# CCIG-Champalimaud/adell-mri

Hardware: AMD Instinct MI355X
Metric: volumes/sec 3D U-Net 128^3 2-ch seg (train step: fwd+loss+bwd+SGD) (higher is better)
Workload: dtype f32 (f16x3 split MFMA, fp32 accumulate); 1 GPU; BASELINE configs[1]: u-net-3d-resnet.yaml UNetPL, 2x128^3, batch 2/GPU, dice+focal, SGD-Nesterov; per_gpu_batch=2, parallelism=dp1, yaml=configs/u-net-3d-resnet.yaml, built_by=parse_config_unet -> get_segmentation_network('unet'), gradient_exchange=none (1 rank)

## Files before the change

adell_mri_amd/_lib.py:

```python
import ctypes
import os

_HERE = os.path.dirname(os.path.abspath(__file__))
LIB_PATH = os.environ.get("ADELL_HIP_LIBRARY") or os.path.join(_HERE, "libadellhip.so")

_lib = None

OK = 0
E_BADARG, E_UNSUPPORTED, E_HIP, E_NOMEM = -1, -2, -3, -4

ACT_IDS = {
    "identity": 0, "swish": 1, "silu": 1, "relu": 2, "leaky_relu": 3, "prelu": 4,
    "gelu": 5, "sigmoid": 6, "tanh": 7, "elu": 8,
}


class AdellHipError(RuntimeError):
    pass


class ConvDesc(ctypes.Structure):
    _fields_ = [(n, ctypes.c_int32) for n in (
        "N", "D", "H", "W", "C0", "C1", "Cout", "KD", "KH", "KW", "SD", "SH", "SW",
        "PD", "PH", "PW", "Do", "Ho", "Wo")]
# ... 65 lines not shown
    "adell_bn_running_update": (_i, [_vp] * 5 + [_i, _l, _f, _f, _vp]),
    "adell_bn_stats_sums": (_i, [_vp, _i, _i, _i, _l, _vp, _vp, ctypes.c_size_t, _vp]),
    "adell_bn_stats_from_sums": (_i, [_vp, _i, _f, _vp, _vp, _vp, _vp, _vp, _f, _vp]),
    "adell_channel_partials_ntiles": (_i, [_l]),
    "adell_channel_partials": (_i, [_vp, _i, _l, _i, _vp, _vp]),
    "adell_norm_act_fwd": (_i, [ctypes.POINTER(NormActDesc), _vp, _vp, _vp, _vp, _vp, _vp, _vp, _vp]),
    "adell_norm_act_mask_bytes": (_l, [ctypes.POINTER(NormActDesc)]),
    "adell_norm_act_fwd_split": (_i, [ctypes.POINTER(NormActDesc)] + [_vp] * 7 + [_i, _vp, _vp]),
    "adell_split_rows_from_f32": (_i, [_vp, _i, _l, _i, _vp, _vp, _vp]),
    "adell_split_rows_to_f32": (_i, [_vp, _i, _l, _i, _vp, _vp, _vp]),
    "adell_conv3d_f16x3_rows_ok": (_i, [ctypes.POINTER(ConvDesc)]),
    "adell_conv3d_bwd_weight_f16x3_rows_ok": (_i, [ctypes.POINTER(ConvDesc)]),
    "adell_conv3d_bwd_weight_f16x3_plan": (_i, [ctypes.POINTER(ConvDesc), _vp]),
    "adell_conv3d_bwd_weight_f16x3_rows": (_i, [ctypes.POINTER(ConvDesc)] + [_vp] * 10
                                           + [ctypes.c_size_t, _vp]),
    "adell_conv3d_fwd_f16x3_rows": (_i, [ctypes.POINTER(ConvDesc)] + [_vp] * 10 + [_i, _vp, _vp]),
    "adell_norm_act_fwd_mask": (_i, [ctypes.POINTER(NormActDesc)] + [_vp] * 9),
    "adell_norm_act_bwd_from_dt": (_i, [ctypes.POINTER(NormActDesc)] + [_vp] * 5 + [_i, _i, _i, _vp, _vp,
                                                                              ctypes.c_size_t, _vp]),
    "adell_conv3d_bwd_data_f16x3_adn_ntiles": (_i, [ctypes.POINTER(ConvDesc)]),
    "adell_conv3d_bwd_data_f16x3_adn": (_i, [ctypes.POINTER(ConvDesc)] + [_vp] * 7
                                        + [ctypes.POINTER(AdnSite), ctypes.POINTER(AdnSite), _vp, _i, _vp]),
    "adell_norm_act_bwd_workspace": (_l, [ctypes.POINTER(NormActDesc)]),
    "adell_norm_act_bwd": (_i, [ctypes.POINTER(NormActDesc)] + [_vp] * 11 + [ctypes.c_size_t, _vp]),
    "adell_norm_act_plan": (_i, [ctypes.POINTER(NormActDesc)] + [_i] * 6 + [_vp]),
    "adell_norm_act_stats_plan": (_i, [_i, _i, _i, _vp]),
    "adell_norm_act_bwd_sums": (_i, [ctypes.POINTER(NormActDesc)] + [_vp] * 11 + [ctypes.c_size_t, _vp]),
    "adell_norm_act_bwd_apply_sums": (_i, [ctypes.POINTER(NormActDesc)] + [_vp] * 10
                                      + [ctypes.c_size_t, _vp]),
    "adell_norm_act_bwd_lowrank": (_i, [ctypes.POINTER(NormActDesc), _vp, _vp, _vp, _i, _vp, _vp, _vp,
# ... 185 lines not shown
    "adell_lesion_candidates_capacity": (_l, [_i] * 6),
    "adell_lesion_candidates": (_i, [_vp, _l, _i, _i, _i, _i, _f, _f] + [_i] * 5 + [_vp] * 6
                                + [_l, ctypes.POINTER(ctypes.c_int), _vp, _l, _vp]),
    "adell_item_stats_workspace": (_l, [_i, _l]),
    "adell_item_stats": (_i, [_vp, _i, _l, _vp, _vp, ctypes.c_size_t, _vp]),
    "adell_aug_intensity": (_i, [_vp, _vp, _i, _l, _vp, ctypes.c_uint64, ctypes.c_uint32, _vp]),
    "adell_affine_sample": (_i, [_vp, _vp, _i, _i, _i, _i, _i, _vp, _i, _i, _vp]),
    "adell_axis_filter": (_i, [_vp, _vp, _i, _i, _i, _i, _i, _i, _vp, _i, _vp]),
    "adell_bias_field": (_i, [_vp, _vp, _i, _i, _i, _i, _i, _vp, _vp]),
    "adell_axis_lut_sample": (_i, [_vp, _vp, _i, _i, _i, _i, _i, _vp, _i, _vp]),
    "adell_dw_mfma_ok": (_i, [_i] * 8 + [_vp, _vp]),
    "adell_dw_dense_ok": (_i, [_i] * 8 + [_vp, _vp]),
    "adell_dw_wgrad_mfma_ok": (_i, [_i] * 8 + [_vp, _vp]),
    "adell_dwconv3d_plan": (_i, [_i] * 11 + [_vp]),
    "adell_wgrad_zring_plan": (_i, [_i] * 16 + [_vp]),
    "adell_rowscale_fwd": (_i, [_vp] * 5 + [_i, _i, _vp]),
    "adell_rowscale_bwd": (_i, [_vp] * 8 + [_i, _i, _vp]),
    "adell_window_ndhwc": (_i, [_vp, _vp] + [_i] * 11 + [_vp]),
    "adell_gibbs_workspace": (_l, [_i, _i, _i, _i, _i]),
    "adell_gibbs_lowpass": (_i, [_vp, _vp, _i, _i, _i, _i, _i, _vp, _vp, ctypes.c_size_t, _vp]),
    "adell_gather_nd": (_i, [_vp, _vp, _i, _vp, _vp, _vp, _i, _vp, _vp, _vp, _vp]),
    "adell_layernorm_rows_fwd": (_i, [_vp, _l, _i, _i, _l, _l, _vp, _vp, _f, _vp, _vp, _vp, _vp]),
    "adell_layernorm_rows_bwd_workspace": (_l, [_l, _i]),
    "adell_layernorm_rows_bwd": (_i, [_vp, _vp, _vp, _vp, _vp, _l, _i, _i, _l, _l, _vp, _l, _l,
                                      _vp, _vp, _vp, ctypes.c_size_t, _vp]),
    "adell_winattn_fwd": (_i, [_vp, _vp, _vp, _l, _l, _vp, _vp, _i, _l, _i, _i, _i, _i, _f, _f,
                               ctypes.c_ulong, ctypes.c_uint, _vp, _vp, _vp]),
    "adell_winattn_bwd": (_i, [_vp, _vp, _vp, _l, _l, _vp, _vp, _i, _vp, _vp, _vp, _l, _i, _i, _i,
                               _i, _f, _f, ctypes.c_ulong, ctypes.c_uint, _vp, _vp, _vp, _vp, _vp]),
    "adell_gemm_f32_workspace_floats": (_l, [_i, _i, _i]),
# ... 73 lines not shown
```

adell_mri_amd/csrc/common.h:

```cpp
#pragma once
#include <hip/hip_runtime.h>
#include <stdint.h>
#include <stdio.h>
#include "../../include/adell_hip.h"

typedef float f32x16 __attribute__((ext_vector_type(16)));
typedef float f32x4 __attribute__((ext_vector_type(4)));

#define ADELL_WAVE 64
#define ADELL_GLOBAL __attribute__((address_space(1)))

void adell_set_error(const char* fmt, ...);

struct AdellTuning {
  int igemm_nospec;
  int igemm_no8;
  int no_splitk;
  int wgrad_nozring;
  int attn_nomfma;
  int dw_nomfma;
  int dw_wgrad_nomfma;
  int wgrad_no16;
  int igemm_no16;
  int gemm_norows;
// ... 19 lines not shown
      adell_set_error("%s:%d: %s -> %s", __FILE__, __LINE__, #expr,            \
                      hipGetErrorString(_e));                                  \
      return ADELL_E_HIP;                                                      \
    }                                                                          \
  } while (0)

#define ADELL_REQUIRE(cond, ...)                                               \
  do {                                                                         \
    if (!(cond)) {                                                             \
      adell_set_error(__VA_ARGS__);                                            \
      return ADELL_E_BADARG;                                                   \
    }                                                                          \
  } while (0)

constexpr int kAdellLdsPerCu = 160 * 1024;

template <auto Kern, typename... Args>
static int adell_launch(dim3 grid, dim3 block, size_t lds, hipStream_t st, const Args&... args) {
  static const hipError_t attr = [] {
    hipFuncAttributes fa;
    const hipError_t e = hipFuncGetAttributes(&fa, reinterpret_cast<const void*>(Kern));
    if (e != hipSuccess) return e;
    return hipFuncSetAttribute(reinterpret_cast<const void*>(Kern),
                               hipFuncAttributeMaxDynamicSharedMemorySize,
                               kAdellLdsPerCu - (int)fa.sharedSizeBytes);
  }();
  if (attr != hipSuccess) {
    adell_set_error("%s: raising the dynamic LDS limit -> %s", __PRETTY_FUNCTION__,
                    hipGetErrorString(attr));
    return ADELL_E_HIP;
  }
  hipLaunchKernelGGL(Kern, grid, block, lds, st, args...);
  const hipError_t e = hipGetLastError();
  if (e != hipSuccess) {
    adell_set_error("%s: launch -> %s", __PRETTY_FUNCTION__, hipGetErrorString(e));
    return ADELL_E_HIP;
  }
  return ADELL_OK;
}

int adell_cu_count();
// ... 125 lines not shown
```

adell_mri_amd/csrc/conv3d.hip:

```cpp
#include "conv_igemm.h"
#include "conv_igemm_f16.h"

#ifdef ADELL_DEBUG
__device__ unsigned long long* adell_g_stamps = nullptr;
extern "C" int adell_debug_set_stamps(void* device_buffer) {
  ADELL_CHECK_HIP(hipMemcpyToSymbol(HIP_SYMBOL(adell_g_stamps), &device_buffer, sizeof(void*)));
  return ADELL_OK;
}
#endif

struct ConvTile {
  int cfg;
  int BM, BN;
  int lTX, lTY, lTZ;
};

static void adell_shape_brick(int BM, int Wo, int Ho, int Do, int* lx, int* ly,
                              int* lz) {
  int bits = adell_ilog2(BM);
  int cap[3] = {adell_ilog2(Wo), adell_ilog2(Ho), adell_ilog2(Do)};
  int l[3] = {0, 0, 0};
  int pref[3] = {3, 3, 2};
  for (int pass = 0; pass < 2 && bits > 0; ++pass) {
    bool progress = true;
// ... 352 lines not shown
  int rows_ok;
  int adn_rows;
  int stat_rows;
  dim3 grid;
};

static bool adell_is_3s1(const ConvArgs& a) {
  return a.KD == 3 && a.KH == 3 && a.KW == 3 && a.SD == 1 && a.SH == 1 && a.SW == 1 && a.UPS == 1 &&
         a.UPSY == 1 && a.UPSZ == 1 && a.shuffle == 0;
}

static bool adell_item_below_4g(const ConvArgs& a) {
  return (size_t)a.D * a.H * a.W * (a.C0 > a.C1 ? a.C0 : a.C1) < ((size_t)1 << 30);
}

static int adell_plan_tile_f16(const ConvArgs& a, int N, ConvPlanF16* p) {
  ConvTile t = adell_pick_tile(N, a.Do, a.Ho, a.Wo, a.Cout, g_conv_force_cfg);
  const bool is3s1 = adell_is_3s1(a);
  if (g_conv_force_cfg < 0 && adell_conv_zring16_ok(&a)) {
    int seglen = 0, nseg = 0;
    adell_conv_zring16_segments(N, a.Do, a.Ho, a.Wo, &seglen, &nseg);
    t.cfg = 8;
    t.BM = 64;
    t.BN = 16;
    t.lTX = 3; t.lTY = 3; t.lTZ = 0;
    p->tile = t;
    p->brick = {adell_cdiv(a.Wo, 8), adell_cdiv(a.Ho, 8), nseg, 10, 10, seglen, 100};
    p->GKH = 3;
    p->lds = 0;
    return ADELL_OK;
// ... 37 lines not shown
    const int next = t.cfg == 0 ? 2 : t.cfg == 1 ? 3 : 6;
    if (t.cfg == next || g_conv_force_cfg >= 0) break;
    t = adell_pick_tile(N, a.Do, a.Ho, a.Wo, a.Cout, next);
  }
  if (lds > 160 * 1024) {
    adell_set_error("conv f16x3: LDS need %zu B exceeds 160 KiB (k=%d stride=%d)", lds, a.KW, a.SW);
    return ADELL_E_UNSUPPORTED;
  }
  if (t.cfg == 1 && !retiled && is3s1 && t.lTX == 3 && t.lTY == 3 && t.lTZ == 2 && a.Do >= 8 &&
      a.C0 % 16 == 0 && a.C1 % 16 == 0 && adell_item_below_4g(a) && g_conv_force_cfg < 0 &&
      !g_adell_tune.igemm_nospec && !g_adell_tune.igemm_no8) {
    t.cfg = 4;
    t.BM = 512;
    t.lTZ = 3;
    p->brick = adell_brick(a, t);
    lds = (size_t)1000 * 64 + (size_t)7 * 32 * 64 + 64;
  }
  if (a.shuffle != 0 && a.KD == 1 && a.KH == 1 && a.KW == 1 && a.Cout >= 128 &&
      g_conv_force_cfg < 0 && !g_adell_tune.igemm_nospec) {
    t.cfg = 5;
    t.BM = 64;
    t.BN = 256;
    adell_shape_brick(64, a.Wo, a.Ho, a.Do, &t.lTX, &t.lTY, &t.lTZ);
    p->brick = adell_brick(a, t);
    p->GKH = 1;
    lds = (size_t)p->brick.VP * 64 + (size_t)256 * 64 + 64;
    if (lds < (size_t)1 * 256 * 2 * sizeof(float)) lds = (size_t)256 * 2 * sizeof(float);
  }
  p->tile = t;
  p->lds = lds;
  return ADELL_OK;
// ... 504 lines not shown
```

adell_mri_amd/csrc/conv_wgrad_f16.hip:

```cpp
#include "conv_wgrad_host.h"

typedef _Float16 half8 __attribute__((ext_vector_type(8)));
typedef _Float16 half4 __attribute__((ext_vector_type(4)));
typedef __fp16 fp16x4 __attribute__((__vector_size__(4 * sizeof(__fp16))));

__device__ __forceinline__ half8 adell_tr_frag(const char* base, int off, int step) {
  typedef __attribute__((address_space(3))) fp16x4* lds_p;
  const fp16x4 lo4 = __builtin_amdgcn_ds_read_tr16_b64_v4f16((lds_p)(base + off));
  const fp16x4 hi4 = __builtin_amdgcn_ds_read_tr16_b64_v4f16((lds_p)(base + off + step));
  half8 r;
  r[0] = (_Float16)lo4[0]; r[1] = (_Float16)lo4[1]; r[2] = (_Float16)lo4[2]; r[3] = (_Float16)lo4[3];
  r[4] = (_Float16)hi4[0]; r[5] = (_Float16)hi4[1]; r[6] = (_Float16)hi4[2]; r[7] = (_Float16)hi4[3];
  return r;
}

struct WgradF16Args {
  const float* x0;
  const float* x1;
  const float* dy;
  float* ws;
  float* wsdb;
  const unsigned* xmax;
  const unsigned* ymax;
  int N, D, H, W;
// ... 498 lines not shown
  a.PD = d.PD; a.PH = d.PH; a.PW = d.PW;
  a.Do = d.Do; a.Ho = d.Ho; a.Wo = d.Wo;
  a.lTY = p.lTY; a.ntx = p.ntx; a.nty = p.nty; a.HX = p.HX; a.HY = p.HY;
  a.GKH = p.GKH; a.NGY = p.NGY;
  a.TCI = p.TCI; a.TCO = p.TCO; a.nci = p.nci; a.nco = p.nco; a.R = p.R;
  a.ksplit = p.ksplit;
  a.vecx = (d.C0 % 4 == 0) && (d.C1 % 4 == 0) && (((uintptr_t)x0 & 15) == 0) &&
           (((uintptr_t)x1 & 15) == 0);
  a.vecy = (d.Cout % 4 == 0) && (((uintptr_t)dy & 15) == 0);
  return r.inst->launch(a, r.grid, p.lds, st);
}

static int adell_wgrad_f16_run(const adell_conv3d_desc& d, const float* x0, const float* x1,
                               const float* dy, float* out, float* db, const uint32_t* xmax_in,
                               const uint32_t* ymax_in, void* ws, size_t ws_bytes, hipStream_t st,
                               const int* xk0 = nullptr, const int* xk1 = nullptr) {
  WgradRoute r;
  const int prc = adell_wgrad_route(d, &r);
  ADELL_REQUIRE((!xk0 && !xk1) || r.rows_ok,
                "wgrad f16x3: this problem does not take split-row sources "
                "(adell_conv3d_bwd_weight_f16x3_rows_ok)");
  if (prc != ADELL_OK) return prc;
  if (r.route == ADELL_WGRAD_SMALL)
    return adell_wgrad_small(&d, x0, x1, dy, out, db, ws, ws_bytes, st);
  const int Cin = d.C0 + d.C1, Cout = d.Cout, ntap = d.KD * d.KH * d.KW;
  const size_t need = adell_wgrad_f16_ws(r.R, d);
  ADELL_REQUIRE(ws != nullptr && ws_bytes >= need, "wgrad f16x3: workspace too small (%zu < %zu)",
                ws_bytes, need);
  float* slabs = (float*)ws;
  float* wsdb = slabs + (size_t)r.R * ntap * Cin * Cout;
  unsigned* amax = reinterpret_cast<unsigned*>(wsdb + (size_t)r.R * Cout);
// ... 2 lines not shown
  auto blocks_for = [](long n) { long b = (n / 4 + 255) / 256; return (int)(b > 2048 ? 2048 : (b < 1 ? 1 : b)); };
  if (!xmax_in || !ymax_in) ADELL_CHECK_HIP(hipMemsetAsync(amax, 0, 4 * sizeof(unsigned), st));
  if (!xmax_in) {
    if (!xk0)
      hipLaunchKernelGGL(adell_absmax2_kernel, dim3(blocks_for(nx0)), dim3(256), 0, st, x0, nx0, amax);
    if (d.C1 > 0 && !xk1)
      hipLaunchKernelGGL(adell_absmax2_kernel, dim3(blocks_for(nx1)), dim3(256), 0, st, x1, nx1, amax);
  }
  if (!ymax_in)
    hipLaunchKernelGGL(adell_absmax2_kernel, dim3(blocks_for(ny)), dim3(256), 0, st, dy, ny, amax + 1);
  const unsigned* xmax = xmax_in ? xmax_in : amax;
  const unsigned* ymax = ymax_in ? ymax_in : amax + 1;
  float* dbs = db ? wsdb : nullptr;
  int rc;
  if (r.route == ADELL_WGRAD_ZRING32 || r.route == ADELL_WGRAD_ZRING16)
    rc = adell_wgrad_zring_launch(d, r.zr, x0, x1, dy, slabs, dbs, xmax, ymax, st, xk0, xk1);
  else if (r.route == ADELL_WGRAD_S2)
    rc = adell_wgrad_s2_launch(d, r.s2, x0, dy, slabs, dbs, xmax, ymax, st);
  else
    rc = adell_wgrad_plane_launch(d, r, x0, x1, dy, slabs, dbs, xmax, ymax, st);
  if (rc != ADELL_OK) return rc;
  return adell_wgrad_reduce_launch(slabs, out, r.R, ntap, Cin, Cout, dbs, db, st);
}

extern "C" long adell_conv3d_bwd_weight_f16x3_workspace(const adell_conv3d_desc* d) {
  if (!d) return ADELL_E_BADARG;
  WgradRoute r;
  if (adell_wgrad_route(*d, &r) != ADELL_OK) return ADELL_E_UNSUPPORTED;
  return adell_wgrad_f16_workspace(*d, r);
}

// ... 18 lines not shown
    for (int i = 0; i < 8; ++i) out[16 + i] = v[i];
  }
  WgradPlan p32;
  if (r.route != ADELL_WGRAD_SMALL && adell_wgrad_plan(*d, &p32) == ADELL_OK) out[24] = p32.maxj_inst;
  return ADELL_OK;
}

extern "C" int adell_conv3d_bwd_weight_f16x3(const adell_conv3d_desc* d, const float* x0,
                                             const float* x1, const float* dy, float* dw,
                                             float* db, const uint32_t* x_absmax,
                                             const uint32_t* dy_absmax, void* workspace,
                                             size_t workspace_bytes, void* stream) {
  ADELL_REQUIRE(d && x0 && dy && dw, "conv_bwd_weight_f16x3: null pointer");
  ADELL_REQUIRE(d->C1 == 0 || x1, "conv_bwd_weight_f16x3: C1 > 0 needs x1");
  return adell_wgrad_f16_run(*d, x0, x1, dy, dw, db, x_absmax, dy_absmax, workspace,
                             workspace_bytes, (hipStream_t)stream);
}

extern "C" int adell_conv3d_bwd_weight_f16x3_rows_ok(const adell_conv3d_desc* d) {
  WgradRoute r;
  return d && adell_wgrad_route(*d, &r) == ADELL_OK && r.rows_ok ? 1 : 0;
}

extern "C" int adell_conv3d_bwd_weight_f16x3_rows(const adell_conv3d_desc* d, const void* x0,
                                                  const int* xk0, const void* x1, const int* xk1,
                                                  const float* dy, float* dw, float* db,
                                                  const uint32_t* x_absmax,
                                                  const uint32_t* dy_absmax, void* workspace,
                                                  size_t workspace_bytes, void* stream) {
  ADELL_REQUIRE(d && x0 && dy && dw, "conv_bwd_weight_f16x3_rows: null pointer");
  ADELL_REQUIRE(d->C1 == 0 || x1, "conv_bwd_weight_f16x3_rows: C1 > 0 needs x1");
  ADELL_REQUIRE(xk0 || xk1, "conv_bwd_weight_f16x3_rows: no split-row source");
  return adell_wgrad_f16_run(*d, (const float*)x0, (const float*)x1, dy, dw, db, x_absmax,
                             dy_absmax, workspace, workspace_bytes, (hipStream_t)stream, xk0, xk1);
}
```

adell_mri_amd/csrc/conv_wgrad_host.h:

```cpp
#pragma once
#include "common.h"

struct WgradZrPlan {
  int ntx, nty, nseg, seglen, nci, nco, R, t16;
};
bool adell_wgrad_zring_plan_desc(const adell_conv3d_desc& d, WgradZrPlan& p);
int adell_wgrad_zring_launch(const adell_conv3d_desc& d, const WgradZrPlan& p, const float* x0,
                             const float* x1, const float* dy, float* slabs, float* wsdb,
                             const unsigned* xmax, const unsigned* ymax, hipStream_t st,
                             const int* xk0, const int* xk1);

struct WgradS2Plan {
  int ntx, nty, ntz, nbricks, blocks, R;
};
bool adell_wgrad_s2_plan(const adell_conv3d_desc& d, WgradS2Plan& p);
int adell_wgrad_s2_launch(const adell_conv3d_desc& d, const WgradS2Plan& p, const float* x,
                          const float* dy, float* slabs, float* wsdb, const unsigned* xmax,
                          const unsigned* ymax, hipStream_t st);

struct WgradF16Plan {
  int lTY, HX, HY, TCI, TCO, nci, nco, maxj, R, ntx, nty, GKH, NGY, ksplit;
  size_t lds;
};

struct WgradPlan {
// ... 14 lines not shown
```

adell_mri_amd/csrc/conv_wgrad_zring.hip:

```cpp
#include "conv_wgrad_host.h"

typedef _Float16 zr_half8 __attribute__((ext_vector_type(8)));
typedef _Float16 zr_half4 __attribute__((ext_vector_type(4)));
typedef __fp16 zr_fp16x4 __attribute__((__vector_size__(4 * sizeof(__fp16))));

__device__ __forceinline__ zr_half8 adell_zr_frag(const char* p) {
  typedef __attribute__((address_space(3))) zr_fp16x4* lds_p;
  const zr_fp16x4 lo4 = __builtin_amdgcn_ds_read_tr16_b64_v4f16((lds_p)(p));
  const zr_fp16x4 hi4 = __builtin_amdgcn_ds_read_tr16_b64_v4f16((lds_p)(p + 4 * 32));
  zr_half8 r;
  r[0] = (_Float16)lo4[0]; r[1] = (_Float16)lo4[1]; r[2] = (_Float16)lo4[2]; r[3] = (_Float16)lo4[3];
  r[4] = (_Float16)hi4[0]; r[5] = (_Float16)hi4[1]; r[6] = (_Float16)hi4[2]; r[7] = (_Float16)hi4[3];
  return r;
}

struct WgradZrArgs {
  const float* x0;
  const float* x1;
  const float* dy;
  float* ws;
  float* wsdb;
  const unsigned* xmax;
  const unsigned* ymax;
  const int* xk0;
// ... 557 lines not shown
  p.R = (int)(nunits < target ? nunits : target);
  return true;
}

extern "C" int adell_wgrad_zring_plan(int N, int D, int H, int W, int C0, int C1, int Cout, int KD,
                                      int KH, int KW, int SD, int SH, int SW, int Do, int Ho, int Wo,
                                      int* plan) {
  const adell_conv3d_desc d = {N, D, H, W, C0, C1, Cout, KD, KH, KW, SD, SH, SW, 0, 0, 0, Do, Ho, Wo};
  WgradZrPlan p;
  if (!adell_wgrad_zring_plan_desc(d, p)) return 0;
  const int v[8] = {p.ntx, p.nty, p.nseg, p.seglen, p.nci, p.nco, p.R, p.t16};
  for (int i = 0; i < 8; ++i) plan[i] = v[i];
  return 1;
}

int adell_wgrad_zring_launch(const adell_conv3d_desc& d, const WgradZrPlan& p, const float* x0,
                             const float* x1, const float* dy, float* slabs, float* wsdb,
                             const unsigned* xmax, const unsigned* ymax, hipStream_t st,
                             const int* xk0, const int* xk1) {
  WgradZrArgs a = {};
  a.x0 = x0; a.x1 = x1; a.dy = dy; a.ws = slabs; a.wsdb = wsdb; a.xmax = xmax; a.ymax = ymax;
  a.xk0 = xk0; a.xk1 = xk1;
  a.N = d.N; a.D = d.D; a.H = d.H; a.W = d.W; a.C0 = d.C0; a.C1 = d.C1; a.Cin = d.C0 + d.C1;
  a.Cout = d.Cout;
  a.PD = d.PD; a.PH = d.PH; a.PW = d.PW; a.Do = d.Do; a.Ho = d.Ho; a.Wo = d.Wo;
  a.ntx = p.ntx; a.nty = p.nty; a.nseg = p.nseg; a.seglen = p.seglen;
  a.nci = p.nci; a.nco = p.nco; a.R = p.R;
  a.dbg = g_adell_tune.zr_dbg;
  const dim3 grid((unsigned)p.R, (unsigned)(p.nci * p.nco));
  if (p.t16) {
    const size_t lds16 = 2 * (ZR_SLOTS * (size_t)Z16_XPLANE + 2 * (size_t)Z16_YPLANE);
    hipLaunchKernelGGL(adell_conv_wgrad_zring16_kernel, grid, dim3(256), lds16, st, a);
    ADELL_CHECK_HIP(hipGetLastError());
    return ADELL_OK;
  }
  const size_t lds = ZR_SLOTS * (size_t)ZR_PLANE + 2 * (size_t)ZR_YBUF;
  return adell_launch<adell_conv_wgrad_zring_kernel>(grid, dim3(256), lds, st, a);
}
```

adell_mri_amd/functional.py:

```python
import collections
import ctypes
import itertools
import os
import weakref

import numpy as np
import torch
import torch.distributed as dist

from . import _lib, ops

_dropout_counter = itertools.count(1)

CONV_PRECISION = os.environ.get("ADELL_CONV_PRECISION", "f16x3")
FLAGS = {"s2class_always": bool(os.environ.get("ADELL_S2CLASS_ALWAYS")),
         "no_s2class": bool(os.environ.get("ADELL_NO_S2CLASS")),
         "no_fold": bool(os.environ.get("ADELL_NO_FOLD")),
         "no_adn_fuse": bool(os.environ.get("ADELL_NO_ADN_FUSE")),
         "no_lowrank": bool(os.environ.get("ADELL_NO_LOWRANK")),
         "wgrad_stream": os.environ.get("ADELL_WGRAD_STREAM", "1") != "0",
         "no_rows": bool(os.environ.get("ADELL_NO_ROWS")),
         "no_pointwise_gemm": bool(os.environ.get("ADELL_NO_POINTWISE_GEMM")),
         "no_seq_attention": bool(os.environ.get("ADELL_NO_SEQ_ATTENTION")),
         "no_mlp_fuse": not bool(os.environ.get("ADELL_MLP_FUSE")),
         "mlp_min_elems": int(os.environ.get("ADELL_MLP_MIN_ELEMS", str(1 << 20))),
         "no_cinfold_wgrad_f16": bool(os.environ.get("ADELL_NO_CINFOLD_WGRAD_F16"))}


def set_conv_precision(mode):
    global CONV_PRECISION
    if mode not in ("f16x3", "fp32"):
        raise ValueError("conv precision must be 'f16x3' or 'fp32'")
    CONV_PRECISION = mode
    _sync_dw_precision()

# ... 533 lines not shown
                    if site is not None:
                        site.fused, site.part, site.poff = True, part, poff
            else:
                fused = add0 is not None and C1 == 0 and f16x3
                dx0, dx1 = ops.conv3d_bwd_data(dy, wpb, in_size, C0, C1, k, stride, padding,
                                               amax=dy_amax, add0=add0 if fused else None)
                if fused:
                    add0 = None
        elif route is not None:
            raise ValueError(f"conv3d: unknown backward-data route {route!r}")
        dx0 = dx0 if need[0] else None
        dx1 = dx1 if x1 is not None and need[1] else None
        want_db = has_bias and need[3]
        wroute = conv3d_wgrad_route(call.route, need[2], want_db)

        def weight_grads():
            db = None
            if wroute == "conv1_small":
                dw, db = ops.conv1_small_bwd_weight(x0, x1, dy, want_db)
            elif wroute.startswith("cinfold"):
                dw, db = ops.conv_cinfold_bwd_weight(x0, dy, padding, want_db,
                                                     f16x3=wroute == "cinfold_f16x3")
            elif wroute.startswith("igemm"):
                dw = ops.conv3d_bwd_weight(x0, dy, k, stride, padding, x1=x1, want_db=want_db,
                                           f16x3=wroute == "igemm_f16x3",
                                           x_amax=None if amax is None else amax[0:1],
                                           dy_amax=dy_amax, rows0=ctx.rows[0], rows1=ctx.rows[1])
                if want_db:
                    dw, db = dw
            elif wroute == "bias_only":
                return None, ops.bias_grad(dy)
            else:
                raise ValueError(f"conv3d: unknown weight-gradient route {wroute!r}")
            return (dw.view(weight.shape) if need[2] else None), db

        if wroute is not None:
            dw, db = (side_run(weight_grads, (x0, x1, dy))
                      if _side_ok(wref.obj, ctx.bias_ref.obj) else weight_grads())
        if add0 is not None and dx0 is not None:
            dx0 = dx0 + add0
        if dx0 is not None and call.carry_x0 is not None:
            call.carry_x0.grad, dx0 = dx0, None
        if dx1 is not None and call.carry_cat is not None:
            call.carry_cat.grad, dx1 = dx1, None
        if has_res and need[4]:
            if call.carry_out is not None:
                call.carry_out.grad = dy
            else:
                dres = dy
        return dx0, dx1, dw, db, dres, None, None


# ... 1694 lines not shown
```

adell_mri_amd/ops.py:

```python
import collections
import ctypes
import functools
import math
import os

import numpy as np
import torch

from . import _lib
from ._lib import ACT_IDS, AdellHipError, ConvDesc, NormActDesc, check


class KernelTimer:

    def __init__(self, only=None):
        self.records = []
        self._agg = None
        self.only = None if only is None else set(only)
        self.active = True

    def start(self):
        e = torch.cuda.Event(enable_timing=True)
        e.record()
        return e
# ... 650 lines not shown

def conv3d_bwd_weight_plan(N, in_size, C0, C1, Cout, kernel, stride, padding):
    d = make_conv_desc(N, tuple(in_size), C0, C1, Cout, kernel, stride, padding)
    out = (ctypes.c_int * 25)()
    rc = _lib.lib().adell_conv3d_bwd_weight_f16x3_plan(ctypes.byref(d), out)
    if rc == _lib.E_UNSUPPORTED:
        return None
    check(rc)
    o = list(out)
    route = WGRAD_ROUTES[o[0]]
    return WgradPlan(route, o[1], o[2] + (o[3] << 31), bool(o[4]),
                     tuple(o[5:8]) if route == "plane" else None, o[8], o[9], o[10], o[11], o[12],
                     tuple(o[13:16]), tuple(o[16:24]) if route.startswith("zring") else None, o[24])


def conv3d_bwd_weight(x0, dy, kernel, stride, padding, x1=None, want_db=False, f16x3=False,
                      x_amax=None, dy_amax=None, rows0=None, rows1=None):
    _require_cuda(x0, x1, dy)
    if rows0 is not None or rows1 is not None:
        ok = f16x3 and conv3d_bwd_weight_rows_ok(
            x0.shape[0], tuple(x0.shape[2:]), x0.shape[1], 0 if x1 is None else x1.shape[1],
            dy.shape[1], kernel, stride, padding)
        if not ok:
            ROWS_FALLBACKS[0] += 1
            if rows0 is not None:
                x0, rows0 = rows_to_f32(x0, rows0), None
            if rows1 is not None:
                x1, rows1 = rows_to_f32(x1, rows1), None
    x0, dy = ndhwc(x0), ndhwc(dy)
    N, C0, D, H, W = x0.shape
    C1 = 0
    if x1 is not None:
# ... 2 lines not shown
    Cout = dy.shape[1]
    k = _triple(kernel)
    d = make_conv_desc(N, (D, H, W), C0, C1, Cout, kernel, stride, padding)
    assert (d.Do, d.Ho, d.Wo) == tuple(dy.shape[2:])
    L = _lib.lib()
    wsfn, fn, name = ((L.adell_conv3d_bwd_weight_f16x3_workspace, L.adell_conv3d_bwd_weight_f16x3,
                       "adell_conv_wgrad_f16_kernel") if f16x3 else
                      (L.adell_conv3d_bwd_weight_workspace, L.adell_conv3d_bwd_weight,
                       "adell_conv_wgrad_kernel"))
    nbytes = wsfn(ctypes.byref(d))
    if nbytes < 0:
        check(int(nbytes))
    ws = _workspace(nbytes, x0.device)
    dw = torch.empty((Cout, C0 + C1, *k), device=x0.device, dtype=torch.float32)
    db = torch.empty((Cout,), device=x0.device, dtype=torch.float32) if want_db else None
    if rows0 is not None or rows1 is not None:
        check(_timed(name, _conv_flops(d), lambda: L.adell_conv3d_bwd_weight_f16x3_rows(
            ctypes.byref(d), _ptr(x0), None if rows0 is None else _ptr(rows0.xk), _ptr(x1),
            None if rows1 is None else _ptr(rows1.xk), _ptr(dy), _ptr(dw), _ptr(db), _ptr(x_amax),
            _ptr(dy_amax), _ptr(ws), ws.numel() * 4, _stream()), _conv_tag(d, "wgrad"),
                     _conv_bytes(d)))
    elif f16x3:
        check(_timed(name, _conv_flops(d), lambda: fn(
            ctypes.byref(d), _ptr(x0), _ptr(x1), _ptr(dy), _ptr(dw), _ptr(db), _ptr(x_amax),
            _ptr(dy_amax), _ptr(ws), ws.numel() * 4, _stream()), _conv_tag(d, "wgrad"),
                     _conv_bytes(d)))
    else:
        check(_timed(name, _conv_flops(d), lambda: fn(
            ctypes.byref(d), _ptr(x0), _ptr(x1), _ptr(dy), _ptr(dw), _ptr(db), _ptr(ws),
            ws.numel() * 4, _stream()), _conv_tag(d, "wgrad"), _conv_bytes(d)))
    return (dw, db) if want_db else dw


def bias_grad(dy):
    _require_cuda(dy)
    dy = ndhwc(dy)
    C = dy.shape[1]
    rows = dy.numel() // C
    nbytes = _lib.lib().adell_bias_grad_workspace(rows, C)
    ws = _workspace(nbytes, dy.device)
# ... 2678 lines not shown
```

include/adell_hip.h:

```cpp
#ifndef ADELL_HIP_H
#define ADELL_HIP_H

#include <stddef.h>
#include <stdint.h>

#ifdef __cplusplus
extern "C" {
#endif
#if defined(__GNUC__) || defined(__clang__)
#pragma GCC visibility push(default)
#endif

#define ADELL_OK 0
#define ADELL_E_BADARG (-1)
#define ADELL_E_UNSUPPORTED (-2)
#define ADELL_E_HIP (-3)
#define ADELL_E_NOMEM (-4)

#define ADELL_ABI_VERSION 2

enum {
  ADELL_ACT_IDENTITY = 0,
  ADELL_ACT_SILU = 1,
  ADELL_ACT_RELU = 2,
// ... 111 lines not shown
int adell_conv3d_bwd_weight(const adell_conv3d_desc* d, const float* x0,
                            const float* x1, const float* dy, float* dw, float* db,
                            void* workspace, size_t workspace_bytes, void* stream);

long adell_conv3d_bwd_weight_f16x3_workspace(const adell_conv3d_desc* d);
int adell_conv3d_bwd_weight_f16x3(const adell_conv3d_desc* d, const float* x0,
                                  const float* x1, const float* dy, float* dw, float* db,
                                  const uint32_t* x_absmax, const uint32_t* dy_absmax,
                                  void* workspace, size_t workspace_bytes, void* stream);
int adell_conv3d_bwd_weight_f16x3_rows_ok(const adell_conv3d_desc* d);
int adell_conv3d_bwd_weight_f16x3_rows(const adell_conv3d_desc* d, const void* x0, const int* xk0,
                                       const void* x1, const int* xk1, const float* dy, float* dw,
                                       float* db, const uint32_t* x_absmax,
                                       const uint32_t* dy_absmax, void* workspace,
                                       size_t workspace_bytes, void* stream);
#define ADELL_WGRAD_SMALL 0
#define ADELL_WGRAD_ZRING32 1
#define ADELL_WGRAD_ZRING16 2
#define ADELL_WGRAD_S2 3
#define ADELL_WGRAD_PLANE 4
int adell_conv3d_bwd_weight_f16x3_plan(const adell_conv3d_desc* d, int* out);

long adell_bias_grad_workspace(long rows, int C);
int adell_bias_grad(const float* dy, long rows, int C, float* db, void* workspace,
                    size_t workspace_bytes, void* stream);

int adell_convtranspose3d_fwd(int N, int D, int H, int W, int Cin, int Cout, int FD, int FH,
                              int FW, const float* x, const float* w_packed, const float* bias,
                              float* y, void* stream);
int adell_convtranspose3d_bwd_data(int N, int D, int H, int W, int Cin, int Cout, int FD,
// ... 607 lines not shown
int adell_dw_wgrad_mfma_ok(int N, int C, int D, int H, int W, int KD, int KH, int KW, const float* x,
                           const float* dy);

#define ADELL_DW_GENERIC 0
#define ADELL_DW_DENSE 1
#define ADELL_DW_MFMA 2
#define ADELL_DW_MFMA_STREAM 3
#define ADELL_DW_ZRING 4
#define ADELL_DW_TILE 5
#define ADELL_DW_WGRAD_MFMA 6
int adell_dwconv3d_plan(int pass, int N, int C, int D, int H, int W, int KD, int KH, int KW,
                        int a_aligned, int b_aligned, long* out);

int adell_wgrad_zring_plan(int N, int D, int H, int W, int C0, int C1, int Cout, int KD, int KH,
                           int KW, int SD, int SH, int SW, int Do, int Ho, int Wo, int* plan);

int adell_rowscale_fwd(const float* gamma, const float* W, const float* b, float* W2, float* b2, int C,
                       int K, void* stream);
int adell_rowscale_bwd(const float* gamma, const float* W, const float* b, const float* dW2,
                       const float* db2, float* dgamma, float* dW, float* db, int C, int K,
                       void* stream);

int adell_window_ndhwc(const float* in, float* out, int N, int C, int Di, int Hi, int Wi, int Do, int Ho,
                       int Wo, int od, int oh, int ow, void* stream);

long adell_gibbs_workspace(int N, int D, int H, int W, int C);
int adell_gibbs_lowpass(const float* x, float* out, int N, int D, int H, int W, int C,
                        const float* radius, void* workspace, size_t workspace_bytes, void* stream);

#if defined(__GNUC__) || defined(__clang__)
// ... 7 lines not shown
```

Before: 62.44 volumes/s.

## Pad z-ring wgrad LDS so side-stream wgrad leaves room for concurrent conv

When the weight-gradient z-ring kernel runs on the side stream, it now requests enough dynamic LDS to cap itself at one block per CU. That reserves LDS for the largest specialised forward/data conv kernel to co-reside on the same CU. The aim is more real overlap between the side-stream wgrad and the main-stream data-gradient convolutions, instead of wgrad blocks filling the CUs. The cost is halved wgrad occupancy, gated by a heuristic on block count and steps and limited to the non-t16 kernel.

```diff
diff --git a/adell_mri_amd/_lib.py b/adell_mri_amd/_lib.py
--- a/adell_mri_amd/_lib.py
+++ b/adell_mri_amd/_lib.py
@@ -103,6 +103,10 @@
     "adell_conv3d_bwd_weight_f16x3_plan": (_i, [ctypes.POINTER(ConvDesc), _vp]),
     "adell_conv3d_bwd_weight_f16x3_rows": (_i, [ctypes.POINTER(ConvDesc)] + [_vp] * 10
                                            + [ctypes.c_size_t, _vp]),
+    "adell_conv3d_bwd_weight_f16x3_share": (_i, [ctypes.POINTER(ConvDesc)] + [_vp] * 8
+                                            + [ctypes.c_size_t, _vp, _i]),
+    "adell_conv3d_bwd_weight_f16x3_rows_share": (_i, [ctypes.POINTER(ConvDesc)] + [_vp] * 10
+                                                 + [ctypes.c_size_t, _vp, _i]),
     "adell_conv3d_fwd_f16x3_rows": (_i, [ctypes.POINTER(ConvDesc)] + [_vp] * 10 + [_i, _vp, _vp]),
     "adell_norm_act_fwd_mask": (_i, [ctypes.POINTER(NormActDesc)] + [_vp] * 9),
     "adell_norm_act_bwd_from_dt": (_i, [ctypes.POINTER(NormActDesc)] + [_vp] * 5 + [_i, _i, _i, _vp, _vp,
@@ -318,6 +322,8 @@
     "adell_dw_wgrad_mfma_ok": (_i, [_i] * 8 + [_vp, _vp]),
     "adell_dwconv3d_plan": (_i, [_i] * 11 + [_vp]),
     "adell_wgrad_zring_plan": (_i, [_i] * 16 + [_vp]),
+    "adell_wgrad_zring_share_plan": (_i, [ctypes.POINTER(ConvDesc), _i, _vp]),
+    "adell_wgrad_zring_occupancy": (_i, [ctypes.POINTER(ConvDesc), _i]),
     "adell_rowscale_fwd": (_i, [_vp] * 5 + [_i, _i, _vp]),
     "adell_rowscale_bwd": (_i, [_vp] * 8 + [_i, _i, _vp]),
     "adell_window_ndhwc": (_i, [_vp, _vp] + [_i] * 11 + [_vp]),
diff --git a/adell_mri_amd/csrc/common.h b/adell_mri_amd/csrc/common.h
--- a/adell_mri_amd/csrc/common.h
+++ b/adell_mri_amd/csrc/common.h
@@ -57,9 +57,13 @@
   } while (0)
 
 constexpr int kAdellLdsPerCu = 160 * 1024;
-
-template <auto Kern, typename... Args>
-static int adell_launch(dim3 grid, dim3 block, size_t lds, hipStream_t st, const Args&... args) {
+constexpr size_t kAdellLdsGranule = 320 * 4;
+constexpr size_t adell_lds_alloc(size_t bytes) {
+  return (bytes + kAdellLdsGranule - 1) / kAdellLdsGranule * kAdellLdsGranule;
+}
+
+template <auto Kern>
+static hipError_t adell_raise_lds_limit() {
   static const hipError_t attr = [] {
     hipFuncAttributes fa;
     const hipError_t e = hipFuncGetAttributes(&fa, reinterpret_cast<const void*>(Kern));
@@ -68,6 +72,12 @@
                                hipFuncAttributeMaxDynamicSharedMemorySize,
                                kAdellLdsPerCu - (int)fa.sharedSizeBytes);
   }();
+  return attr;
+}
+
+template <auto Kern, typename... Args>
+static int adell_launch(dim3 grid, dim3 block, size_t lds, hipStream_t st, const Args&... args) {
+  const hipError_t attr = adell_raise_lds_limit<Kern>();
   if (attr != hipSuccess) {
     adell_set_error("%s: raising the dynamic LDS limit -> %s", __PRETTY_FUNCTION__,
                     hipGetErrorString(attr));
diff --git a/adell_mri_amd/csrc/conv3d.hip b/adell_mri_amd/csrc/conv3d.hip
--- a/adell_mri_amd/csrc/conv3d.hip
+++ b/adell_mri_amd/csrc/conv3d.hip
@@ -390,6 +390,12 @@
   return (size_t)a.D * a.H * a.W * (a.C0 > a.C1 ? a.C0 : a.C1) < ((size_t)1 << 30);
 }
 
+constexpr size_t kConvSpec3Lds = (size_t)1000 * 64 + (size_t)7 * 32 * 64 + 64;
+constexpr size_t kConvSpec1LdsMax = (size_t)600 * 64 + (size_t)9 * 64 * 64 + 64;
+size_t adell_conv_f16_spec_lds_max() {
+  return kConvSpec3Lds > kConvSpec1LdsMax ? kConvSpec3Lds : kConvSpec1LdsMax;
+}
+
 static int adell_plan_tile_f16(const ConvArgs& a, int N, ConvPlanF16* p) {
   ConvTile t = adell_pick_tile(N, a.Do, a.Ho, a.Wo, a.Cout, g_conv_force_cfg);
   const bool is3s1 = adell_is_3s1(a);
@@ -457,7 +463,7 @@
     t.BM = 512;
     t.lTZ = 3;
     p->brick = adell_brick(a, t);
-    lds = (size_t)1000 * 64 + (size_t)7 * 32 * 64 + 64;
+    lds = kConvSpec3Lds;
   }
   if (a.shuffle != 0 && a.KD == 1 && a.KH == 1 && a.KW == 1 && a.Cout >= 128 &&
       g_conv_force_cfg < 0 && !g_adell_tune.igemm_nospec) {
diff --git a/adell_mri_amd/csrc/conv_wgrad_f16.hip b/adell_mri_amd/csrc/conv_wgrad_f16.hip
--- a/adell_mri_amd/csrc/conv_wgrad_f16.hip
+++ b/adell_mri_amd/csrc/conv_wgrad_f16.hip
@@ -536,7 +536,7 @@
 static int adell_wgrad_f16_run(const adell_conv3d_desc& d, const float* x0, const float* x1,
                                const float* dy, float* out, float* db, const uint32_t* xmax_in,
                                const uint32_t* ymax_in, void* ws, size_t ws_bytes, hipStream_t st,
-                               const int* xk0 = nullptr, const int* xk1 = nullptr) {
+                               const int* xk0, const int* xk1, int share) {
   WgradRoute r;
   const int prc = adell_wgrad_route(d, &r);
   ADELL_REQUIRE((!xk0 && !xk1) || r.rows_ok,
@@ -569,7 +569,8 @@
   float* dbs = db ? wsdb : nullptr;
   int rc;
   if (r.route == ADELL_WGRAD_ZRING32 || r.route == ADELL_WGRAD_ZRING16)
-    rc = adell_wgrad_zring_launch(d, r.zr, x0, x1, dy, slabs, dbs, xmax, ymax, st, xk0, xk1);
+    rc = adell_wgrad_zring_launch(d, r.zr, x0, x1, dy, slabs, dbs, xmax, ymax, st, xk0, xk1,
+                                  share);
   else if (r.route == ADELL_WGRAD_S2)
     rc = adell_wgrad_s2_launch(d, r.s2, x0, dy, slabs, dbs, xmax, ymax, st);
   else
@@ -618,7 +619,25 @@
   ADELL_REQUIRE(d && x0 && dy && dw, "conv_bwd_weight_f16x3: null pointer");
   ADELL_REQUIRE(d->C1 == 0 || x1, "conv_bwd_weight_f16x3: C1 > 0 needs x1");
   return adell_wgrad_f16_run(*d, x0, x1, dy, dw, db, x_absmax, dy_absmax, workspace,
-                             workspace_bytes, (hipStream_t)stream);
+                             workspace_bytes, (hipStream_t)stream, nullptr, nullptr,
+                             ADELL_WGRAD_SHARE_NONE);
+}
+
+static bool adell_wgrad_share_ok(int share) {
+  return share == ADELL_WGRAD_SHARE_NONE || share == ADELL_WGRAD_SHARE_AUTO ||
+         share == ADELL_WGRAD_SHARE_ALWAYS;
+}
+
+extern "C" int adell_conv3d_bwd_weight_f16x3_share(const adell_conv3d_desc* d, const float* x0,
+                                                   const float* x1, const float* dy, float* dw,
+                                                   float* db, const uint32_t* x_absmax,
+                                                   const uint32_t* dy_absmax, void* workspace,
+                                                   size_t workspace_bytes, void* stream, int share) {
+  ADELL_REQUIRE(d && x0 && dy && dw, "conv_bwd_weight_f16x3_share: null pointer");
+  ADELL_REQUIRE(d->C1 == 0 || x1, "conv_bwd_weight_f16x3_share: C1 > 0 needs x1");
+  ADELL_REQUIRE(adell_wgrad_share_ok(share), "conv_bwd_weight_f16x3_share: unknown hint %d", share);
+  return adell_wgrad_f16_run(*d, x0, x1, dy, dw, db, x_absmax, dy_absmax, workspace,
+                             workspace_bytes, (hipStream_t)stream, nullptr, nullptr, share);
 }
 
 extern "C" int adell_conv3d_bwd_weight_f16x3_rows_ok(const adell_conv3d_desc* d) {
@@ -636,5 +655,23 @@
   ADELL_REQUIRE(d->C1 == 0 || x1, "conv_bwd_weight_f16x3_rows: C1 > 0 needs x1");
   ADELL_REQUIRE(xk0 || xk1, "conv_bwd_weight_f16x3_rows: no split-row source");
   return adell_wgrad_f16_run(*d, (const float*)x0, (const float*)x1, dy, dw, db, x_absmax,
-                             dy_absmax, workspace, workspace_bytes, (hipStream_t)stream, xk0, xk1);
-}
+                             dy_absmax, workspace, workspace_bytes, (hipStream_t)stream, xk0, xk1,
+                             ADELL_WGRAD_SHARE_NONE);
+}
+
+extern "C" int adell_conv3d_bwd_weight_f16x3_rows_share(const adell_conv3d_desc* d, const void* x0,
+                                                        const int* xk0, const void* x1,
+                                                        const int* xk1, const float* dy, float* dw,
+                                                        float* db, const uint32_t* x_absmax,
+                                                        const uint32_t* dy_absmax, void* workspace,
+                                                        size_t workspace_bytes, void* stream,
+                                                        int share) {
+  ADELL_REQUIRE(d && x0 && dy && dw, "conv_bwd_weight_f16x3_rows_share: null pointer");
+  ADELL_REQUIRE(d->C1 == 0 || x1, "conv_bwd_weight_f16x3_rows_share: C1 > 0 needs x1");
+  ADELL_REQUIRE(xk0 || xk1, "conv_bwd_weight_f16x3_rows_share: no split-row source");
+  ADELL_REQUIRE(adell_wgrad_share_ok(share), "conv_bwd_weight_f16x3_rows_share: unknown hint %d",
+                share);
+  return adell_wgrad_f16_run(*d, (const float*)x0, (const float*)x1, dy, dw, db, x_absmax,
+                             dy_absmax, workspace, workspace_bytes, (hipStream_t)stream, xk0, xk1,
+                             share);
+}
diff --git a/adell_mri_amd/csrc/conv_wgrad_host.h b/adell_mri_amd/csrc/conv_wgrad_host.h
--- a/adell_mri_amd/csrc/conv_wgrad_host.h
+++ b/adell_mri_amd/csrc/conv_wgrad_host.h
@@ -5,10 +5,16 @@
   int ntx, nty, nseg, seglen, nci, nco, R, t16;
 };
 bool adell_wgrad_zring_plan_desc(const adell_conv3d_desc& d, WgradZrPlan& p);
+struct WgradZrShare {
+  int per_cu;
+  size_t lds, room;
+};
+WgradZrShare adell_wgrad_zring_share(const adell_conv3d_desc& d, const WgradZrPlan& p, int share);
+size_t adell_conv_f16_spec_lds_max();
 int adell_wgrad_zring_launch(const adell_conv3d_desc& d, const WgradZrPlan& p, const float* x0,
                              const float* x1, const float* dy, float* slabs, float* wsdb,
                              const unsigned* xmax, const unsigned* ymax, hipStream_t st,
-                             const int* xk0, const int* xk1);
+                             const int* xk0, const int* xk1, int share);
 
 struct WgradS2Plan {
   int ntx, nty, ntz, nbricks, blocks, R;
diff --git a/adell_mri_amd/csrc/conv_wgrad_zring.hip b/adell_mri_amd/csrc/conv_wgrad_zring.hip
--- a/adell_mri_amd/csrc/conv_wgrad_zring.hip
+++ b/adell_mri_amd/csrc/conv_wgrad_zring.hip
@@ -595,10 +595,66 @@
   return 1;
 }
 
+constexpr long kZrShareMinSteps = 96;
+static size_t adell_wgrad_zring_lds(int t16) {
+  return t16 ? 2 * (ZR_SLOTS * (size_t)Z16_XPLANE + 2 * (size_t)Z16_YPLANE)
+             : ZR_SLOTS * (size_t)ZR_PLANE + 2 * (size_t)ZR_YBUF;
+}
+
+WgradZrShare adell_wgrad_zring_share(const adell_conv3d_desc& d, const WgradZrPlan& p, int share) {
+  WgradZrShare s = {p.t16 ? 3 : 2, adell_wgrad_zring_lds(p.t16), 0};
+  const long blocks = (long)p.R * p.nci * p.nco;
+  const long nunits = (long)d.N * p.ntx * p.nty * p.nseg;
+  const long steps = (nunits + p.R - 1) / p.R * p.seglen;
+  if (!p.t16 && (share == ADELL_WGRAD_SHARE_ALWAYS ||
+                 (share == ADELL_WGRAD_SHARE_AUTO && blocks > adell_cu_count() &&
+                  steps >= kZrShareMinSteps))) {
+    size_t want = adell_lds_alloc(kAdellLdsPerCu / 2 + 1);
+    if (want < s.lds) want = s.lds;
+    if (2 * adell_lds_alloc(want) > (size_t)kAdellLdsPerCu &&
+        adell_lds_alloc(want) + adell_lds_alloc(adell_conv_f16_spec_lds_max()) <= (size_t)kAdellLdsPerCu) {
+      s.per_cu = 1;
+      s.lds = want;
+    }
+  }
+  s.room = kAdellLdsPerCu - s.per_cu * adell_lds_alloc(s.lds);
+  return s;
+}
+
+extern "C" int adell_wgrad_zring_share_plan(const adell_conv3d_desc* d, int share, int* out) {
+  WgradZrPlan p;
+  if (!d || !out || !adell_wgrad_zring_plan_desc(*d, p)) return 0;
+  const WgradZrShare s = adell_wgrad_zring_share(*d, p, share);
+  const int v[11] = {p.ntx, p.nty, p.nseg, p.seglen, p.nci, p.nco, p.R, p.t16,
+                     s.per_cu, (int)s.lds, (int)s.room};
+  for (int i = 0; i < 11; ++i) out[i] = v[i];
+  return 1;
+}
+
+extern "C" int adell_wgrad_zring_occupancy(const adell_conv3d_desc* d, int share) {
+  ADELL_REQUIRE(d, "wgrad_zring_occupancy: null pointer");
+  WgradZrPlan p;
+  if (!adell_wgrad_zring_plan_desc(*d, p)) {
+    adell_set_error("wgrad_zring_occupancy: the z-ring kernel does not serve this problem");
+    return ADELL_E_UNSUPPORTED;
+  }
+  const WgradZrShare s = adell_wgrad_zring_share(*d, p, share);
+  int n = 0;
+  if (p.t16) {
+    ADELL_CHECK_HIP(hipOccupancyMaxActiveBlocksPerMultiprocessor(&n, adell_conv_wgrad_zring16_kernel,
+                                                                 256, s.lds));
+  } else {
+    ADELL_CHECK_HIP(adell_raise_lds_limit<adell_conv_wgrad_zring_kernel>());
+    ADELL_CHECK_HIP(hipOccupancyMaxActiveBlocksPerMultiprocessor(&n, adell_conv_wgrad_zring_kernel,
+                                                                 256, s.lds));
+  }
+  return n;
+}
+
 int adell_wgrad_zring_launch(const adell_conv3d_desc& d, const WgradZrPlan& p, const float* x0,
                              const float* x1, const float* dy, float* slabs, float* wsdb,
                              const unsigned* xmax, const unsigned* ymax, hipStream_t st,
-                             const int* xk0, const int* xk1) {
+                             const int* xk0, const int* xk1, int share) {
   WgradZrArgs a = {};
   a.x0 = x0; a.x1 = x1; a.dy = dy; a.ws = slabs; a.wsdb = wsdb; a.xmax = xmax; a.ymax = ymax;
   a.xk0 = xk0; a.xk1 = xk1;
@@ -609,12 +665,11 @@
   a.nci = p.nci; a.nco = p.nco; a.R = p.R;
   a.dbg = g_adell_tune.zr_dbg;
   const dim3 grid((unsigned)p.R, (unsigned)(p.nci * p.nco));
+  const size_t lds = adell_wgrad_zring_share(d, p, share).lds;
   if (p.t16) {
-    const size_t lds16 = 2 * (ZR_SLOTS * (size_t)Z16_XPLANE + 2 * (size_t)Z16_YPLANE);
-    hipLaunchKernelGGL(adell_conv_wgrad_zring16_kernel, grid, dim3(256), lds16, st, a);
+    hipLaunchKernelGGL(adell_conv_wgrad_zring16_kernel, grid, dim3(256), lds, st, a);
     ADELL_CHECK_HIP(hipGetLastError());
     return ADELL_OK;
   }
-  const size_t lds = ZR_SLOTS * (size_t)ZR_PLANE + 2 * (size_t)ZR_YBUF;
   return adell_launch<adell_conv_wgrad_zring_kernel>(grid, dim3(256), lds, st, a);
 }
diff --git a/adell_mri_amd/functional.py b/adell_mri_amd/functional.py
--- a/adell_mri_amd/functional.py
+++ b/adell_mri_amd/functional.py
@@ -19,6 +19,7 @@
          "no_adn_fuse": bool(os.environ.get("ADELL_NO_ADN_FUSE")),
          "no_lowrank": bool(os.environ.get("ADELL_NO_LOWRANK")),
          "wgrad_stream": os.environ.get("ADELL_WGRAD_STREAM", "1") != "0",
+         "no_wgrad_share": bool(os.environ.get("ADELL_NO_WGRAD_SHARE")),
          "no_rows": bool(os.environ.get("ADELL_NO_ROWS")),
          "no_pointwise_gemm": bool(os.environ.get("ADELL_NO_POINTWISE_GEMM")),
          "no_seq_attention": bool(os.environ.get("ADELL_NO_SEQ_ATTENTION")),
@@ -582,7 +583,7 @@
         want_db = has_bias and need[3]
         wroute = conv3d_wgrad_route(call.route, need[2], want_db)
 
-        def weight_grads():
+        def weight_grads(on_side=False):
             db = None
             if wroute == "conv1_small":
                 dw, db = ops.conv1_small_bwd_weight(x0, x1, dy, want_db)
@@ -593,7 +594,8 @@
                 dw = ops.conv3d_bwd_weight(x0, dy, k, stride, padding, x1=x1, want_db=want_db,
                                            f16x3=wroute == "igemm_f16x3",
                                            x_amax=None if amax is None else amax[0:1],
-                                           dy_amax=dy_amax, rows0=ctx.rows[0], rows1=ctx.rows[1])
+                                           dy_amax=dy_amax, rows0=ctx.rows[0], rows1=ctx.rows[1],
+                                           share=on_side and not FLAGS["no_wgrad_share"])
                 if want_db:
                     dw, db = dw
             elif wroute == "bias_only":
@@ -603,7 +605,7 @@
             return (dw.view(weight.shape) if need[2] else None), db
 
         if wroute is not None:
-            dw, db = (side_run(weight_grads, (x0, x1, dy))
+            dw, db = (side_run(lambda: weight_grads(on_side=True), (x0, x1, dy))
                       if _side_ok(wref.obj, ctx.bias_ref.obj) else weight_grads())
         if add0 is not None and dx0 is not None:
             dx0 = dx0 + add0
diff --git a/adell_mri_amd/ops.py b/adell_mri_amd/ops.py
--- a/adell_mri_amd/ops.py
+++ b/adell_mri_amd/ops.py
@@ -688,8 +688,20 @@
                      tuple(o[13:16]), tuple(o[16:24]) if route.startswith("zring") else None, o[24])
 
 
+WgradSharePlan = collections.namedtuple("WgradSharePlan", "zring blocks_per_cu lds room")
+
+
+def conv3d_bwd_weight_share_plan(N, in_size, C0, C1, Cout, kernel, stride, padding, share):
+    d = make_conv_desc(N, tuple(in_size), C0, C1, Cout, kernel, stride, padding)
+    out = (ctypes.c_int * 11)()
+    if not _lib.lib().adell_wgrad_zring_share_plan(ctypes.byref(d), int(share), out):
+        return None
+    o = list(out)
+    return WgradSharePlan(tuple(o[:8]), o[8], o[9], o[10])
+
+
 def conv3d_bwd_weight(x0, dy, kernel, stride, padding, x1=None, want_db=False, f16x3=False,
-                      x_amax=None, dy_amax=None, rows0=None, rows1=None):
+                      x_amax=None, dy_amax=None, rows0=None, rows1=None, share=False):
     _require_cuda(x0, x1, dy)
     if rows0 is not None or rows1 is not None:
         ok = f16x3 and conv3d_bwd_weight_rows_ok(
@@ -722,16 +734,21 @@
     ws = _workspace(nbytes, x0.device)
     dw = torch.empty((Cout, C0 + C1, *k), device=x0.device, dtype=torch.float32)
     db = torch.empty((Cout,), device=x0.device, dtype=torch.float32) if want_db else None
+    hint = (int(share),) if share and f16x3 else ()
     if rows0 is not None or rows1 is not None:
-        check(_timed(name, _conv_flops(d), lambda: L.adell_conv3d_bwd_weight_f16x3_rows(
+        rows_fn = (L.adell_conv3d_bwd_weight_f16x3_rows_share if hint
+                   else L.adell_conv3d_bwd_weight_f16x3_rows)
+        check(_timed(name, _conv_flops(d), lambda: rows_fn(
             ctypes.byref(d), _ptr(x0), None if rows0 is None else _ptr(rows0.xk), _ptr(x1),
             None if rows1 is None else _ptr(rows1.xk), _ptr(dy), _ptr(dw), _ptr(db), _ptr(x_amax),
-            _ptr(dy_amax), _ptr(ws), ws.numel() * 4, _stream()), _conv_tag(d, "wgrad"),
+            _ptr(dy_amax), _ptr(ws), ws.numel() * 4, _stream(), *hint), _conv_tag(d, "wgrad"),
                      _conv_bytes(d)))
     elif f16x3:
+        if hint:
+            fn = L.adell_conv3d_bwd_weight_f16x3_share
         check(_timed(name, _conv_flops(d), lambda: fn(
             ctypes.byref(d), _ptr(x0), _ptr(x1), _ptr(dy), _ptr(dw), _ptr(db), _ptr(x_amax),
-            _ptr(dy_amax), _ptr(ws), ws.numel() * 4, _stream()), _conv_tag(d, "wgrad"),
+            _ptr(dy_amax), _ptr(ws), ws.numel() * 4, _stream(), *hint), _conv_tag(d, "wgrad"),
                      _conv_bytes(d)))
     else:
         check(_timed(name, _conv_flops(d), lambda: fn(
diff --git a/include/adell_hip.h b/include/adell_hip.h
--- a/include/adell_hip.h
+++ b/include/adell_hip.h
@@ -149,6 +149,20 @@
                                        float* db, const uint32_t* x_absmax,
                                        const uint32_t* dy_absmax, void* workspace,
                                        size_t workspace_bytes, void* stream);
+#define ADELL_WGRAD_SHARE_NONE 0
+#define ADELL_WGRAD_SHARE_AUTO 1
+#define ADELL_WGRAD_SHARE_ALWAYS 2
+int adell_conv3d_bwd_weight_f16x3_share(const adell_conv3d_desc* d, const float* x0,
+                                        const float* x1, const float* dy, float* dw, float* db,
+                                        const uint32_t* x_absmax, const uint32_t* dy_absmax,
+                                        void* workspace, size_t workspace_bytes, void* stream,
+                                        int share);
+int adell_conv3d_bwd_weight_f16x3_rows_share(const adell_conv3d_desc* d, const void* x0,
+                                             const int* xk0, const void* x1, const int* xk1,
+                                             const float* dy, float* dw, float* db,
+                                             const uint32_t* x_absmax, const uint32_t* dy_absmax,
+                                             void* workspace, size_t workspace_bytes, void* stream,
+                                             int share);
 #define ADELL_WGRAD_SMALL 0
 #define ADELL_WGRAD_ZRING32 1
 #define ADELL_WGRAD_ZRING16 2
@@ -786,6 +800,8 @@
 
 int adell_wgrad_zring_plan(int N, int D, int H, int W, int C0, int C1, int Cout, int KD, int KH,
                            int KW, int SD, int SH, int SW, int Do, int Ho, int Wo, int* plan);
+int adell_wgrad_zring_share_plan(const adell_conv3d_desc* d, int share, int* out);
+int adell_wgrad_zring_occupancy(const adell_conv3d_desc* d, int share);
 
 int adell_rowscale_fwd(const float* gamma, const float* W, const float* b, float* W2, float* b2, int C,
                        int K, void* stream);
```

Measured after the change: 63.36 volumes/s (median of 6 runs). 1.5% higher.
